# cortes-ciriano-lab/DeMethify

Measured on AMD Instinct MI355X. Metric: NMF update iters/sec (1e6 CpG x 256 samples x 16 types), higher is better.
Workload: dtype f64; 1 GPU; headline_1e6x256_12+4; N_cpg=1000000, S_samples=256, n_known=12, n_unknown=4, inner_iters=20, restarts=64, restart_seed=1 + k, restart_placement=k mod n_gpus, parallelism=restart-sharded x1

## Files before the change

### demethify_amd/csrc/dmf_api_solver.hip

```cpp
#include "dmf_api.h"

namespace dmf_api {

using dmf::kSplitInnerSteps;

static int ensure_split_scratch(dmf_solver* s, int n_iter2) {
    dmf_context* ctx = s->ctx;
    if (s->cm == nullptr) HIP_TRY(s->cm.alloc(ctx, (size_t)dmf::u_phase_split_cm_doubles(s->p->N, (int)s->n_u)));
    if (s->beta_cap < n_iter2 || s->beta_tab == nullptr) {
        s->beta_cap = n_iter2 > 0 ? n_iter2 : 1;
        HIP_TRY(s->beta_tab.alloc(ctx, (size_t)s->beta_cap));
    }
    return DMF_OK;
}

int enqueue_u_phase(dmf_solver* s, int n_iter2, dmf::RowKind row) {
    dmf_context* ctx = s->ctx;
    const dmf::ProblemView pv = s->p->view();
    FamilyScope scope(ctx, DMF_KERNEL_ROWPASS);
    switch (row) {
        case dmf::RowKind::CmI8InnerRows:
            DMF_TRY(ensure_split_scratch(s, n_iter2));
            HIP_TRY(dmf::launch_u_phase_split_i8(pv, s->iterate(), n_iter2, s->scratch(), ctx->stream));
            return DMF_OK;
// ... 171 lines not shown
    state->mom_i = 0;
    state->mom_n = n;
}

static double momentum_advance(double& a) {
#pragma clang fp contract(off)
    const double a0 = a;
    const double sq = 4.0 * a0 * a0;
    a = (1.0 + std::sqrt(1.0 + sq)) / 2.0;
    return (a0 - 1.0) / a;
}

static int upload_momentum_rows(dmf_solver* s, int rows, int n) {
    dmf_context* ctx = s->ctx;
    const int stride = 2 + 2 * n;
    if (s->mom_host == nullptr) {
        if (!ctx->pinned_moms.empty()) {
            s->mom_host = ctx->pinned_moms.back();
            ctx->pinned_moms.pop_back();
        } else {
            HIP_TRY(hipHostMalloc((void**)&s->mom_host, (size_t)kMomRows * (2 + 2 * kMomSteps) * sizeof(double)));
        }
        HIP_TRY(s->mom_dev.alloc(ctx, (size_t)kMomRows * (2 + 2 * kMomSteps)));
    }
    double a1 = s->h_state->a1, a2 = s->h_state->a2;
    for (int r = 0; r < rows; ++r) {
        double* row = s->mom_host + (size_t)r * stride;
        for (int t = 0; t < n; ++t) {
            row[2 + t] = momentum_advance(a1);
            row[2 + n + t] = momentum_advance(a2);
        }
        row[0] = a1;
        row[1] = a2;
    }
    HIP_TRY(hipMemcpyAsync(s->mom_dev, s->mom_host, (size_t)rows * stride * sizeof(double), hipMemcpyHostToDevice, ctx->stream));
    hipLaunchKernelGGL(k_set_momentum, dim3(1), dim3(1), 0, ctx->stream, s->state.get(), (const double*)s->mom_dev.get(), stride,
                       rows, n);
    HIP_TRY(hipGetLastError());
    return DMF_OK;
}

__global__ void k_set_tol(SolverState* state, double tol, double band) {
    state->tol = tol;
    state->band = band;
}

constexpr double kConfirmBand = 10.0;
constexpr double kGramCostRelErr = 1e-15;

static double* cost_slot(const dmf_solver* s) {
    return reinterpret_cast<double*>(reinterpret_cast<char*>(s->h_state) + kPinnedStateBytes - 16);
}

static int solver_setup(dmf_solver* s, const double* u0, const double* alpha0, int flags) {
    dmf_context* ctx = s->ctx;
    const dmf_problem* p = s->p;
    const int64_t N = p->N, S = p->S, n_c = p->n_c, n_u = s->n_u, K = n_c + n_u;
    dmf::ShapeKey& key = s->key;
    key.N = N;
    key.S = (int)S;
    key.n_c = (int)n_c;
    key.n_u = (int)n_u;
    key.nd = (p->ND > 0 && p->D16 != nullptr) ? p->ND : 0;
    key.SD = p->SD;
    key.x16 = key.nd > 0 && p->X16 != nullptr;
    key.rowpass_pair = ctx->rowpass_pair;
    key.level = ctx->generic_level;
    key.d_f32_exact = p->d_f32_exact;
    key.rtp_present = n_c == 0 || p->Rtp != nullptr;
    key.v_align = (unsigned)(reinterpret_cast<uintptr_t>(p->V.get()) & 15);
    key.rtp_align = (unsigned)(reinterpret_cast<uintptr_t>(p->Rtp.get()) & 15);
    key.alpha_unit = true;
    s->spec = dmf::select_path(key);
    if ((s->spec.use_v2 || s->spec.use_cm_i8) && !(flags & DMF_INIT_IN_UNIT_RANGE)) {
        bool in_unit = true;
        if (flags & DMF_PTR_DEVICE) {
            double outside = 0.0;
            HIP_TRY(dmf::launch_unit_range_check(alpha0, K * S, ctx->scratch, ctx->scratch + 2048, ctx->stream));
            HIP_TRY(hipMemcpyAsync(&outside, ctx->scratch + 2048, sizeof(double), hipMemcpyDeviceToHost, ctx->stream));
            HIP_TRY(hipStreamSynchronize(ctx->stream));
            in_unit = outside == 0.0;
        } else {
            for (int64_t i = 0; i < K * S; ++i)
                if (!(alpha0[i] >= 0.0 && alpha0[i] <= 1.0)) {
                    in_unit = false;
                    break;
                }
        }
        if (!in_unit) {
            key.alpha_unit = false;
            s->spec = dmf::select_path(key);
        }
    }
    if (!s->spec.supported) return DMF_ERR_UNSUPPORTED;
    s->in_flight = true;
    s->jobs.build((int)n_c, (int)K, [n_c, K](int k, int l) {
        if (l == (int)K && k < (int)n_c) return false;
        return !(l == (int)K && k == (int)K);
    });
    const int n_jobs = s->jobs.n;
    s->slab_doubles = dmf::gram_slab_doubles(N, (int)S, n_jobs);
    if (s->spec.use_gram_spec) {
        const int64_t spec = dmf::gram_u_slab_doubles(N, (int)S, (int)n_c, (int)n_u);
        if (spec > s->slab_doubles) s->slab_doubles = spec;
    }
    if (s->spec.use_gram_mfma) {
        const int64_t need = dmf::gram_mfma_slab_doubles(N, (int)S, n_jobs);
        if (need > s->slab_doubles) s->slab_doubles = need;
    }
    if (s->spec.use_fused) {
        const int64_t spec = dmf::rowpass_fused_slab_doubles(N - (N & 15), (int)S, (int)n_c, (int)n_u) +
                             dmf::gram_u_slab_doubles(16, (int)S, (int)n_c, (int)n_u);
        if (spec > s->slab_doubles) s->slab_doubles = spec;
    }
    if (s->spec.use_v2) {
        const int64_t bu = (int64_t)dmf::rowpass_v2_grid(N, (int)S) * n_u * S;
        if (bu > s->slab_doubles) s->slab_doubles = bu;
    }
    if (s->spec.use_gram_i8) {
        const int64_t bu = (int64_t)dmf::bu_cols_grid(N) * n_u * S;
        if (bu > s->slab_doubles) s->slab_doubles = bu;
        if (s->spec.use_cm_i8) {
            const int64_t bu2 = (int64_t)dmf::u_inner_bu_grid(N, (int)S) * n_u * S;
            if (bu2 > s->slab_doubles) s->slab_doubles = bu2;
        }
    }
    const size_t un = (size_t)N * n_u, an = (size_t)K * S;
    const size_t un_alloc = (un + 1) & ~(size_t)1;
    const size_t gbn = (size_t)(K + 1) * (K + 2) / 2 * S;
    const int nb_alpha = (int)((S + 63) / 64);
    HIP_TRY(s->u.alloc(ctx, un_alloc));
    HIP_TRY(s->u_prev.alloc(ctx, un_alloc));
    if (s->spec.u_path == 2) HIP_TRY(s->u_next.alloc(ctx, un_alloc));
    HIP_TRY(s->alpha.alloc(ctx, an));
    HIP_TRY(s->alpha_prev.alloc(ctx, an));
    HIP_TRY(s->gb.alloc(ctx, gbn));
    HIP_TRY(s->slab.alloc(ctx, (size_t)s->slab_doubles));
    HIP_TRY(s->partials.alloc(ctx, (size_t)2 * (nb_alpha + S)));
    HIP_TRY(s->u2_partials.alloc(ctx, 4096));
    if (s->spec.use_v2 || s->spec.use_gram_i8) {
        s->slab_i8_words = dmf::gram_i8_slab_words(N, p->SD, (int)n_c, (int)n_u);
        HIP_TRY(s->slab_i8.alloc(ctx, (size_t)s->slab_i8_words));
        const size_t acc_words = (size_t)dmf::gram_i8_acc_words((int)S, (int)n_c, (int)n_u);
        HIP_TRY(s->acc_i8.alloc(ctx, acc_words));
        HIP_TRY(hipMemsetAsync(s->acc_i8, 0, acc_words * sizeof(long long), ctx->stream));
    }
    HIP_TRY(s->state.alloc(ctx, 1));
    if (!ctx->pinned_states.empty()) {
        s->h_state = (SolverState*)ctx->pinned_states.back();
        ctx->pinned_states.pop_back();
    } else {
        HIP_TRY(hipHostMalloc((void**)&s->h_state, kPinnedStateBytes));
    }
    const hipMemcpyKind in_kind = (flags & DMF_PTR_DEVICE) ? hipMemcpyDeviceToDevice : hipMemcpyHostToDevice;
    HIP_TRY(hipMemsetAsync(s->state, 0, sizeof(SolverState), ctx->stream));
    HIP_TRY(hipMemsetAsync(s->gb, 0, gbn * sizeof(double), ctx->stream));
    HIP_TRY(hipMemcpyAsync(s->u, u0, un * sizeof(double), in_kind, ctx->stream));
    HIP_TRY(hipMemcpyAsync(s->u_prev, s->u, un * sizeof(double), hipMemcpyDeviceToDevice, ctx->stream));
    HIP_TRY(hipMemcpyAsync(s->alpha, alpha0, an * sizeof(double), in_kind, ctx->stream));
    HIP_TRY(hipMemcpyAsync(s->alpha_prev, s->alpha, an * sizeof(double), hipMemcpyDeviceToDevice, ctx->stream));
    DMF_TRY(s->jobs.upload(ctx));
    HIP_TRY(dmf::launch_scatter_known_block(p->gb_known, s->gb, (int)n_c, (int)K, (int)S, ctx->stream));
    HIP_TRY(dmf::launch_sumsq_f64(s->u, N * n_u, ctx->scratch, &s->state->u_norm2, nullptr, ctx->stream));
    HIP_TRY(dmf::launch_init_state(s->state, p->consts, s->alpha, (int)S, (int)n_c, (int)n_u, ctx->stream));
    if (!(flags & DMF_PTR_DEVICE)) HIP_TRY(hipStreamSynchronize(ctx->stream));
    return DMF_OK;
}

}

using namespace dmf_api;

extern "C" {

int dmf_solver_create(dmf_context* ctx, const dmf_problem* p, const double* u0, const double* alpha0,
                      int64_t n_u, int mode, int flags, dmf_solver** out) {
    DMF_TRY(check_ctx(ctx));
    if (out == nullptr) return DMF_ERR_BAD_ARG;
    *out = nullptr;
    if (p == nullptr || u0 == nullptr || alpha0 == nullptr || n_u < 1) return DMF_ERR_BAD_ARG;
    if (mode != DMF_MODE_PARTIAL && mode != DMF_MODE_UNSUPERVISED) return DMF_ERR_BAD_ARG;
    if (p->n_c + n_u > dmf::kMaxK) return DMF_ERR_UNSUPPORTED;
    SolverPtr s(new (std::nothrow) dmf_solver());
    if (s == nullptr) return DMF_ERR_BAD_ARG;
    s->ctx = ctx;
    s->p = p;
    s->n_u = n_u;
    s->mode = mode;
    DMF_TRY(solver_setup(s.get(), u0, alpha0, flags));
    *out = s.release();
    return DMF_OK;
}

int dmf_solver_step(dmf_solver* s, int64_t n_outer, int64_t n_iter2, double tol,
                    int64_t* iters_done_total, int* converged) {
    if (s == nullptr || n_outer < 0 || n_iter2 < 0 || n_iter2 > (1 << 20)) return DMF_ERR_BAD_ARG;
    dmf_context* ctx = s->ctx;
    DMF_TRY(check_ctx(ctx));
    const dmf_problem* p = s->p;
    const double gram_err = kGramCostRelErr * (double)p->N * (double)p->S * p->h_consts[kDmax] +
                            (s->key.x16 ? p->x16_dev * p->x16_sum : 0.0);
    s->confirm_stops = tol > 0.0 && ctx->stop_confirmation != 2 && (ctx->stop_confirmation == 1 || gram_err >= tol / 20.0);
    hipLaunchKernelGGL(k_set_tol, dim3(1), dim3(1), 0, ctx->stream, s->state.get(), tol, s->confirm_stops ? kConfirmBand : 1.0);
    HIP_TRY(hipGetLastError());
    if (s->cf_pending && tol > 0.0 && n_outer > 0) {
        FamilyScope scope(ctx, DMF_KERNEL_COST);
        HIP_TRY(enqueue_cost(ctx, p->view(), s->u, s->alpha, (int)s->n_u, ctx->scratch + 1024, &s->state->cf));
        s->cf_pending = false;
        s->cf_stream_iter = -2;
    }
    DMF_TRY(fetch_state(s));
    if (s->cf_stream_iter == -2) {
        s->cf_stream = s->h_state->cf;
        s->cf_stream_iter = s->h_state->iters;
    }
    int64_t check_every = s->spec.u_path != 2 ? 8 : 1;
    if (tol == 0.0 && s->spec.u_path != 2) check_every = kMomRows;
    const long long iters0 = s->h_state->iters;
    const dmf::IterationPlan plan = dmf::plan_iteration(s->key, s->spec, (int)n_iter2, s->purity != nullptr);
    const bool use_mom = n_iter2 >= 1 && n_iter2 <= kMomSteps && plan.row == dmf::RowKind::RowpassV2 &&
                         plan.alpha == dmf::AlphaKind::PhaseRow16;
    if (!use_mom && s->h_state->mom_n >= 0) {
        hipLaunchKernelGGL(k_set_momentum, dim3(1), dim3(1), 0, ctx->stream, s->state.get(), (const double*)nullptr, 0, 0, -1);
        HIP_TRY(hipGetLastError());
    }
    while (s->h_state->iters - iters0 < n_outer && s->h_state->done != 1) {
        const int64_t left = n_outer - (s->h_state->iters - iters0);
        const int64_t batch = left < check_every ? left : check_every;
        if (use_mom) DMF_TRY(upload_momentum_rows(s, (int)batch, (int)n_iter2));
        for (int64_t b = 0; b < batch; ++b) DMF_TRY(enqueue_outer_iteration(s, (int)n_iter2));
        DMF_TRY(fetch_state(s));
        if (s->h_state->iters > iters0) s->cf_pending = false;
        if (s->h_state->done == 2) {
            double cs = 0.0;
            DMF_TRY(cost_to_host(ctx, p->view(), s->u, s->alpha, (int)s->n_u, &cs, true));
            bool stop;
            if (s->cf_stream_iter == s->h_state->iters - 1) {
                stop = std::fabs(cs - s->cf_stream) < tol;
                s->n_confirmed += 1;
            } else {
                stop = std::fabs(s->h_state->cf - s->h_state->cf_prev) < tol;
                s->n_unconfirmed += 1;
            }
            s->cf_stream = cs;
            s->cf_stream_iter = s->h_state->iters;
            s->h_state->done = stop ? 1 : 0;
            DMF_TRY(push_state(s));
            check_every = 1;
        } else if (s->spec.u_path != 2 && check_every < 64 && check_every > 1) {
            check_every *= 2;
        }
    }
    if (iters_done_total) *iters_done_total = s->h_state->iters;
    if (converged) *converged = s->h_state->done == 1;
    return DMF_OK;
}

int dmf_solver_set_purity(dmf_solver* s, const double* purity, int flags) {
    if (s == nullptr || purity == nullptr) return DMF_ERR_BAD_ARG;
    dmf_context* ctx = s->ctx;
    DMF_TRY(check_ctx(ctx));
    if (s->mode != DMF_MODE_PARTIAL) return DMF_ERR_BAD_ARG;
    const size_t bytes = (size_t)s->p->S * sizeof(double);
    if (s->purity == nullptr) HIP_TRY(s->purity.alloc(ctx, (size_t)s->p->S));
    const hipMemcpyKind kind = (flags & DMF_PTR_DEVICE) ? hipMemcpyDeviceToDevice : hipMemcpyHostToDevice;
    HIP_TRY(hipMemcpyAsync(s->purity, purity, bytes, kind, ctx->stream));
    HIP_TRY(hipStreamSynchronize(ctx->stream));
    return DMF_OK;
}

int dmf_solver_get(dmf_solver* s, int flags, double* out_u, double* out_alpha, double* out_cost,
                   int64_t* out_iters) {
    if (s == nullptr) return DMF_ERR_BAD_ARG;
    dmf_context* ctx = s->ctx;
    DMF_TRY(check_ctx(ctx));
    const dmf_problem* p = s->p;
    DMF_TRY(export_array(ctx, s->u, (size_t)p->N * s->n_u * sizeof(double), flags, out_u));
    DMF_TRY(export_array(ctx, s->alpha, (size_t)(p->n_c + s->n_u) * p->S * sizeof(double), flags, out_alpha));
    if (s->cf_pending && out_cost != nullptr) {
        FamilyScope scope(ctx, DMF_KERNEL_COST);
        HIP_TRY(enqueue_cost(ctx, p->view(), s->u, s->alpha, (int)s->n_u, ctx->scratch + 1024, &s->state->cf));
        s->cf_pending = false;
    }
    DMF_TRY(fetch_state(s));
    if (out_cost) *out_cost = s->h_state->cf;
    if (out_iters) *out_iters = s->h_state->iters;
    return DMF_OK;
}

int dmf_solver_cost(dmf_solver* s, double* out_cost) {
    if (s == nullptr || out_cost == nullptr) return DMF_ERR_BAD_ARG;
    DMF_TRY(check_ctx(s->ctx));
    return cost_to_host(s->ctx, s->p->view(), s->u, s->alpha, (int)s->n_u, out_cost, true);
}

int dmf_solver_cost_begin(dmf_solver* s) {
    if (s == nullptr) return DMF_ERR_BAD_ARG;
    dmf_context* ctx = s->ctx;
    DMF_TRY(check_ctx(ctx));
    if (s->cost_event == nullptr) {
        if (!ctx->events.empty()) {
            s->cost_event = ctx->events.back();
            ctx->events.pop_back();
        } else {
            HIP_TRY(hipEventCreateWithFlags(&s->cost_event, hipEventDisableTiming));
        }
    }
    DMF_TRY(cost_to_host(ctx, s->p->view(), s->u, s->alpha, (int)s->n_u, cost_slot(s), false));
    HIP_TRY(hipEventRecord(s->cost_event, ctx->stream));
    s->cost_pending = true;
    return DMF_OK;
}

int dmf_solver_cost_end(dmf_solver* s, double* out_cost) {
    if (s == nullptr || out_cost == nullptr || !s->cost_pending) return DMF_ERR_BAD_ARG;
    DMF_TRY(check_ctx(s->ctx));
    HIP_TRY(hipEventSynchronize(s->cost_event));
// ... 77 lines not shown
```

### demethify_amd/csrc/dmf_internal.h

```cpp
#pragma once
#include <hip/hip_runtime.h>
#include <stdint.h>

#include "dmf_select.h"

namespace dmf {

struct SolverState {
    double a1;
    double a2;
    double l_w;
    double l_w_prev;
    double l_h;
    double l_h_prev;
    double dsq;
    double rt_norm2;
    double u_norm2;
    double cf;
    double cf_prev;
    double tol;
    long long iters;
    double band;
    int done;
    int arrive;
    const double* mom;
    int mom_stride, mom_rows, mom_i, mom_n;
};

__device__ __forceinline__ const double* momentum_row(const SolverState* __restrict__ state, int n_iter2) {
    return (state->mom != nullptr && state->mom_n == n_iter2 && state->mom_i < state->mom_rows)
               ? state->mom + (int64_t)state->mom_i * state->mom_stride
               : nullptr;
}

__host__ __device__ inline int tri(int k, int l) { return l * (l + 1) / 2 + k; }

constexpr int kMaxK = 64;
constexpr int kGramChunk = 16;
constexpr int kRowsPerBlockU = 64;

struct GramJobTable {
    const short* k_idx;
    const short* l_idx;
    const int* dst_row;
    int count;
};

struct PercentilePlan {
    long long k_prev, k_next;
    double gamma;
    int from_top;
    int pad;
};

struct ProblemView {
    const double* V = nullptr;
    const double* D = nullptr;
    const unsigned short* D16 = nullptr;
    const unsigned short* X16 = nullptr;
    const signed char* Dt8 = nullptr;
    int64_t plane_stride = 0;
    int SD = 0, ND = 0;
    const double* Rt = nullptr;
    const double* Rtp = nullptr;
    int64_t N = 0;
    int S = 0, n_c = 0;
    unsigned v_align() const { return (unsigned)(reinterpret_cast<uintptr_t>(V) & 15); }
    ProblemView rows(int64_t first, int64_t count) const {
        ProblemView r;
        r.V = V + first * S;
        r.D = D + first * S;
        r.Rt = Rt ? Rt + first * n_c : nullptr;
        r.Rtp = Rtp ? Rtp + first * ((n_c + 3) / 4 * 4) : nullptr;
        r.N = count;
        r.S = S;
        r.n_c = n_c;
        return r;
    }
};

struct IterateView {
    double* u = nullptr;
    double* u_prev = nullptr;
    const double* alpha = nullptr;
    SolverState* state = nullptr;
    int n_u = 0, mode = 0;
    IterateView rows(int64_t first) const {
        IterateView r = *this;
        r.u = u + first * n_u;
        r.u_prev = u_prev + first * n_u;
        return r;
    }
};

struct AlphaView {
    const double* gb = nullptr;
    double* alpha = nullptr;
    double* alpha_prev = nullptr;
    const double* purity = nullptr;
    SolverState* state = nullptr;
    double* partials = nullptr;
    int S = 0, n_c = 0, n_u = 0;
};

struct UScratch {
    double* cm = nullptr;
    double* beta = nullptr;
    double* slab = nullptr;
    double* u2_partials = nullptr;
};


hipError_t launch_convert_counts(const long long* src, double* dst, int64_t n, hipStream_t st);
hipError_t launch_max_f64(const double* x, int64_t n, double* scratch, double* out, hipStream_t st);
hipError_t launch_f32_residual_max(const double* x, int64_t n, double* scratch, double* out, hipStream_t st);
hipError_t launch_int_count_max(const double* x, int64_t n, double* scratch, double* out, hipStream_t st);
hipError_t launch_unit_range_check(const double* x, int64_t n, double* scratch, double* out, hipStream_t st);
hipError_t launch_sumsq_f64(const double* x, int64_t n, double* scratch, double* out,
                            const int* done_flag, hipStream_t st);
hipError_t launch_pad_rows(const double* src, double* dst, int64_t n_rows, int width_src, int width_dst,
                           hipStream_t st);
hipError_t launch_index_range_check(const long long* idx, int64_t n_idx, int64_t n_src, unsigned int* flag, hipStream_t st);
hipError_t launch_gather_rows(const double* src, double* dst, const long long* idx, int64_t n_idx,
                              int64_t width, hipStream_t st);

hipError_t launch_cost(const ProblemView& p, const double* u, const double* alpha, int n_u, double* scratch, double* out,
                       hipStream_t st);

bool cost_cols_supported(int S, int n_c, int n_u);
bool cost_cols2_wide_supported(const ProblemView& p, int n_u);
hipError_t launch_cost_cols2_wide(const ProblemView& p, const double* u, const double* alpha, int n_u, double* scratch,
                                  double* out, hipStream_t st);
int vdv_cols_grid(int64_t N);
hipError_t launch_vdv_cols(const ProblemView& p, double* slab, double* out, hipStream_t st);
hipError_t launch_cost_cols(const ProblemView& p, const double* u, const double* alpha, int n_u, double* scratch, double* out,
                            hipStream_t st);

hipError_t launch_gram(const ProblemView& p, const double* u, int n_u, GramJobTable jobs, double* slab, int64_t slab_doubles,
                       double* gb, const int* done_flag, hipStream_t st);
int64_t gram_slab_doubles(int64_t N, int S, int n_jobs);
hipError_t launch_gram_reduce(const double* slab, int ny, int n_jobs, int S, const int* dst_row,
                              double* gb, const int* done_flag, hipStream_t st);
bool gram_u_supported(int n_c, int n_u);
int64_t gram_u_slab_doubles(int64_t N, int S, int n_c, int n_u);
hipError_t launch_gram_u(const ProblemView& p, const double* u, int n_u, double* slab, const int* done_flag, int* ny_out,
                         hipStream_t st);

hipError_t launch_u_phase_gram(const ProblemView& p, const IterateView& it, int n_iter2, hipStream_t st);
bool u_phase_gram_supported(int S, int n_c, int n_u);
bool u_phase_mfma_supported(int S, int n_c, int n_u);
hipError_t launch_u_phase_mfma(const ProblemView& p, const IterateView& it, int n_iter2, hipStream_t st);
bool rowpass_fused_supported(int S, int n_c, int n_u);
int rowpass_fused_grid(int64_t N, int S);
int64_t rowpass_fused_slab_doubles(int64_t N, int S, int n_c, int n_u);
hipError_t launch_rowpass_fused(const ProblemView& p, const IterateView& it, int n_iter2, const UScratch& scratch,
                                int* grid_out, hipStream_t st);
hipError_t launch_finish_u_norm(const double* u2_partials, int n, SolverState* state, hipStream_t st);
hipError_t launch_u_step_direct(const ProblemView& p, const IterateView& it, double* u_next, int t, hipStream_t st);
bool u_step_direct_supported(int S, int n_c, int n_u);

hipError_t launch_alpha(AlphaKind kind, const AlphaView& a, int n_iter2, hipStream_t st);
hipError_t launch_set_lh(SolverState* state, hipStream_t st);
hipError_t launch_project_simplex(const double* X, double* out, int K, int S, double z,
                                  hipStream_t st);
hipError_t launch_scatter_known_block(const double* gb_known, double* gb, int n_c, int K, int S,
                                      hipStream_t st);
hipError_t launch_init_state(SolverState* state, const double* consts, const double* alpha,
                             int S, int n_c, int n_u, hipStream_t st);

int64_t u_phase_split_cm_doubles(int64_t N, int n_u);
hipError_t launch_u_phase_split(const ProblemView& p, const IterateView& it, int n_iter2, const UScratch& scratch,
                                hipStream_t st);

bool cm_i8_supported(unsigned v_align, int S, int n_c, int n_u, int ND, int SD);
hipError_t launch_cm_i8(const ProblemView& p, const IterateView& it, double* cm, hipStream_t st);
hipError_t launch_u_phase_split_i8(const ProblemView& p, const IterateView& it, int n_iter2, const UScratch& scratch,
                                   hipStream_t st);

bool u_inner_bu_supported(unsigned v_align, int S, int SD, int n_u, int n_iter2);
int u_inner_bu_grid(int64_t N, int S);
hipError_t launch_u_phase_split_i8_bu(const ProblemView& p, const IterateView& it, int n_iter2, const UScratch& scratch,
                                      int* grid_out, hipStream_t st);

bool u_phase_big_supported(int S, int n_c, int n_u, int n_iter2);
hipError_t launch_u_phase_big(const ProblemView& p, const IterateView& it, int n_iter2, hipStream_t st);

hipError_t launch_gram_mfma(const ProblemView& p, const double* u, int n_u, GramJobTable jobs, int n_dense, double* slab,
                            int64_t slab_doubles, const int* done_flag, int* ny_out, hipStream_t st);
int64_t gram_mfma_slab_doubles(int64_t N, int S, int n_jobs);

hipError_t launch_gather_counts_int(const unsigned short* src16, const unsigned short* src_x16, const long long* idx,
                                    int64_t n_idx, int SD, int ND, unsigned short* D16, unsigned short* X16, int64_t N16,
                                    signed char* Dt8, int64_t plane_stride, unsigned int* max_out,
                                    unsigned long long* xsum_out, hipStream_t st);
constexpr double kX16MaxDev = 8.0 * 0x1p-53;
hipError_t launch_build_counts_int(const double* D, const double* V, int64_t N, int S, int ND, unsigned short* D16,
                                   unsigned short* X16, int64_t N16, int SD, signed char* Dt8, int64_t plane_stride,
                                   unsigned long long* x_stats, hipStream_t st);
hipError_t launch_build_dt8(const unsigned short* D16, int64_t N, int SD, int ND, signed char* Dt8, int64_t plane_stride,
                            hipStream_t st);
hipError_t launch_mask_problem(const double* srcV, const double* srcD, const unsigned short* src16,
                               const unsigned short* srcX, const unsigned char* bits, double* dstV, double* dstD,
                               unsigned short* dst16, unsigned short* dstX, unsigned short* W16, int64_t N, int64_t N16, int S,
                               int SD, unsigned long long* stats, hipStream_t st);
hipError_t launch_holdout_weights_f64(const unsigned char* bits, double* W, int64_t N, int S, hipStream_t st);
bool rowpass_v2_supported(int S, int n_c, int n_u, int n_iter2);
int rowpass_v2_grid(int64_t N, int S);
hipError_t launch_rowpass_v2(const ProblemView& p, const IterateView& it, int n_iter2, const UScratch& scratch, int* grid_out,
                             bool pair, bool* paired_out, hipStream_t st);
bool rowpass_v2_pair_fits(int S, int n_u, int n_iter2);
bool gram_i8_supported(int n_c, int n_u, int ND, int64_t N, int SD);
int64_t gram_i8_slab_words(int64_t N, int SD, int n_c, int n_u);
int64_t gram_i8_acc_words(int S, int n_c, int n_u);
bool gram_i8_known_supported(int n_c, int ND, int64_t N, int SD);
int64_t gram_i8_slab_words_nf(int64_t N, int SD, int nf);
int64_t gram_i8_acc_words_nf(int S, int nf, int n_bu);
hipError_t launch_gram_i8(const ProblemView& p, const double* u, int n_u, const short* feat_a, const short* feat_b, int NF,
                          long long* slab, int64_t slab_words, const int* done_flag, int* ny_out, hipStream_t st);
int bu_cols_grid(int64_t N);
hipError_t launch_bu_cols(const ProblemView& p, const double* u, int n_u, double* slab, const int* done_flag,
                          int* n_slabs_out, hipStream_t st, bool* with_vdv = nullptr);
hipError_t launch_gram_v2_reduce(const long long* slab_i8, int ny, int NF, int SD, const double* slab_bu, int n_bu_slabs,
                                 int n_u, int S, long long* acc_words, const int* dst_row, double* gb, const int* done_flag,
                                 const double* u2_partials, int n_u2, SolverState* state, hipStream_t st);

hipError_t launch_percentile_pair(const double* x, int64_t n, int64_t m, PercentilePlan p0, PercentilePlan p1,
                                  double* out0, double* out1, hipStream_t st);
int64_t percentile_max_replicates();

int wls_moments_grid(int64_t N);
int64_t wls_slab_doubles(int64_t N, int S, int K);
hipError_t launch_wls_moments(const ProblemView& p, const double* u, int n_u, int target_dv, double* slab, double* mom,
                              hipStream_t st);
hipError_t launch_nnls_intercept(const double* gb, const double* mom, int K, int S, double* out, int* status, hipStream_t st);

constexpr int kSvdMaxS = 512, kSvdMaxNc = 64, kSvdMaxRank = 64;
constexpr size_t kSvdMaxLds = 160 * 1024;
size_t svd_project_lds_bytes(int S, int rank);
struct SvdColumns {
    double sign[kSvdMaxRank], scale[kSvdMaxRank];
};
bool svd_supported(int S, int n_c, int rank);
int svd_gram_grid(int64_t N, int S);
int64_t svd_gram_slab_doubles(int64_t N, int S);
hipError_t launch_svd_gram(const ProblemView& p, const double* H1, double* slab, int* flags, double* C, hipStream_t st);
int64_t svd_project_slab_doubles(int64_t N, int rank);
hipError_t launch_svd_project(const ProblemView& p, const double* H1, const double* Es, int rank, double* T, double* slab,
                              double* norms, hipStream_t st);
hipError_t launch_svd_finish(double* T, int64_t N, int rank, const SvdColumns& cols, hipStream_t st);

}
```

### demethify_amd/csrc/dmf_kernels_alpha.hip

```cpp
#include "dmf_device.h"
#include "dmf_dispatch.h"
#include "dmf_internal.h"

namespace dmf {

template <int KMAX>
__device__ __forceinline__ void sort_desc(double (&x)[KMAX]) {
#pragma unroll
    for (int k = 2; k <= KMAX; k <<= 1) {
#pragma unroll
        for (int j = k >> 1; j > 0; j >>= 1) {
#pragma unroll
            for (int i = 0; i < KMAX; ++i) {
                const int l = i ^ j;
                if (l > i) {
                    const double lo = fmin(x[i], x[l]), hi = fmax(x[i], x[l]);
                    if ((i & k) == 0) { x[i] = hi; x[l] = lo; }
                    else { x[i] = lo; x[l] = hi; }
                }
            }
        }
    }
}

// ... 573 lines not shown

template <int J>
__device__ __forceinline__ void argmin_step(double& v, int& idx, int k) {
    const double ov = row_xor<J>(v, k);
    const int oi = row_xor<J>(idx, k);
    const bool take = ov < v || (ov == v && oi < idx);
    v = take ? ov : v;
    idx = take ? oi : idx;
}

__global__ __launch_bounds__(64) void k_alpha_frank_wolfe_row16(const double* __restrict__ gb,
                                                                double* __restrict__ alpha,
                                                                const double* __restrict__ purity,
                                                                const SolverState* __restrict__ state, int S, int K,
                                                                int n_u, int max_iter, double* __restrict__ partials) {
    if (state->done) return;
    const int lane = threadIdx.x;
    const int k = lane & 15, grp = lane >> 4, base = grp * 16;
    const int s = blockIdx.x * 4 + grp;
    const bool col_ok = s < S;
    const int sc = col_ok ? s : S - 1;
    const bool row_ok = k < K;
    const int kc = row_ok ? k : K - 1;
    const int n_c = K - n_u;
    const bool known = k < n_c, unknown = row_ok && !known;

    double Grow[16];
#pragma unroll
    for (int l = 0; l < 16; ++l) {
        const int lc = l < K ? l : K - 1;
        const int lo = kc < lc ? kc : lc, hi = kc < lc ? lc : kc;
        const double v = gb[(int64_t)tri(lo, hi) * S + sc];
        Grow[l] = (row_ok && l < K) ? v : 0.0;
    }
    const double bk = row_ok ? gb[(int64_t)tri(kc, K) * S + sc] : 0.0;
    const double pur = purity[sc];
    const double mass = known ? pur : 1.0 - pur;
    double a = row_ok ? alpha[(int64_t)kc * S + sc] : 0.0;

    for (int it = 0; it < max_iter; ++it) {
        double g4[4] = {-bk, 0.0, 0.0, 0.0};
        fmac_rowbcast_seq<0, 16, true, true>(g4, a, Grow);
        const double grad = (g4[0] + g4[1]) + (g4[2] + g4[3]);
        double v1 = known ? grad : INFINITY, v2 = unknown ? grad : INFINITY;
        int i1 = k, i2 = k;
        argmin_step<1>(v1, i1, k); argmin_step<2>(v1, i1, k); argmin_step<4>(v1, i1, k); argmin_step<8>(v1, i1, k);
        argmin_step<1>(v2, i2, k); argmin_step<2>(v2, i2, k); argmin_step<4>(v2, i2, k); argmin_step<8>(v2, i2, k);
        const double gamma = 2.0 / (double)(it + 2);
        const bool at_vertex = (known && k == i1) || (unknown && k == i2);
        const double vertex = at_vertex ? mass : 0.0;
        a = (1.0 - gamma) * a + gamma * vertex;
    }
    if (col_ok && row_ok) alpha[(int64_t)k * S + s] = a;
    double ga = 0.0;
#pragma unroll
    for (int l = 0; l < 16; ++l) ga = fma(Grow[l], __shfl(a, base + l, 64), ga);
    double part = col_ok ? fma(a, ga, -2.0 * a * bk) : 0.0;
    if (col_ok && k == 0) part += gb[(int64_t)tri(K, K) * S + sc];
    const double n2 = (col_ok && unknown) ? a * a : 0.0;
    store_partials(partials, wave_sum(part), wave_sum(n2));
}

template <class F>
static hipError_t dispatch_kmax(int K, F&& f) {
    if (K > 16) return f(std::integral_constant<int, 0>{});
    if (K > 8) return f(std::integral_constant<int, 16>{});
    return K > 4 ? f(std::integral_constant<int, 8>{}) : f(std::integral_constant<int, 4>{});
}

template <int KMAX>
static hipError_t launch_alpha_thread(const AlphaView& a, int n_iter2, hipStream_t st) {
    const int K = a.n_c + a.n_u, nb = (a.S + 63) / 64;
    if constexpr (KMAX > 0) {
        const size_t lds = (size_t)(K + 1) * (K + 2) / 2 * 64 * sizeof(double);
        const int in_lds = lds <= 150 * 1024;
        if (in_lds && lds > 48 * 1024) {
            const hipError_t e = raise_dynamic_lds<k_alpha_phase<KMAX>>(lds);
            if (e != hipSuccess) return e;
        }
        hipLaunchKernelGGL(k_alpha_phase<KMAX>, dim3(nb), dim3(64), in_lds ? lds : 0, st, a.gb, a.alpha, a.alpha_prev, a.state,
                           a.S, K, a.n_u, n_iter2, in_lds, a.partials);
    } else {
        hipLaunchKernelGGL(k_alpha_phase_dyn, dim3(nb), dim3(64), 0, st, a.gb, a.alpha, a.alpha_prev, a.state, a.S, K, a.n_u,
                           n_iter2, a.partials);
    }
    return launch_finish_iteration(a.partials, nb, a.state, n_iter2, st);
}

template <int G>
static hipError_t launch_alpha_lanes(const AlphaView& a, int n_iter2, hipStream_t st) {
    const int nb = (a.S * G + 63) / 64;
    hipLaunchKernelGGL(k_alpha_phase_lanes<G>, dim3(nb), dim3(64), 0, st, a.gb, a.alpha, a.alpha_prev, a.state, a.S,
                       a.n_c + a.n_u, a.n_u, n_iter2, a.partials);
    return launch_finish_iteration(a.partials, nb, a.state, n_iter2, st);
}

hipError_t launch_alpha(AlphaKind kind, const AlphaView& a, int n_iter2, hipStream_t st) {
    const int S = a.S, K = a.n_c + a.n_u, nb4 = (S + 3) / 4, nb64 = (S + 63) / 64;
    if (K < 1 || K > kMaxK) return hipErrorInvalidValue;
    switch (kind) {
        case AlphaKind::PhaseRow16:
            if (K > 16) break;
            hipLaunchKernelGGL(k_alpha_phase_row16, dim3(nb4), dim3(64), 0, st, a.gb, a.alpha, a.alpha_prev, a.state, S, K, a.n_u,
                               n_iter2, a.partials);
            return hipGetLastError();
        case AlphaKind::PhaseLanes:
            if (K <= 16) break;
            return K <= 32 ? launch_alpha_lanes<32>(a, n_iter2, st) : launch_alpha_lanes<64>(a, n_iter2, st);
        case AlphaKind::Phase:
            if (K > 16) break;
            return dispatch_kmax(K, [&](auto kmax) { return launch_alpha_thread<kmax>(a, n_iter2, st); });
        case AlphaKind::PhaseDyn:
            if (K <= 16) break;
            return launch_alpha_thread<0>(a, n_iter2, st);
        case AlphaKind::FrankWolfeRow16:
            if (K > 16 || a.n_c < 1 || a.purity == nullptr) break;
            hipLaunchKernelGGL(k_alpha_frank_wolfe_row16, dim3(nb4), dim3(64), 0, st, a.gb, a.alpha, a.purity, a.state, S, K,
                               a.n_u, n_iter2, a.partials);
            return launch_finish_iteration(a.partials, nb4, a.state, n_iter2, st);
        case AlphaKind::FrankWolfe:
            if (a.purity == nullptr) break;
            hipLaunchKernelGGL(k_alpha_frank_wolfe, dim3(nb64), dim3(64), 0, st, a.gb, a.alpha, a.purity, a.state, S, K, a.n_u,
                               n_iter2, a.partials);
            return launch_finish_iteration(a.partials, nb64, a.state, n_iter2, st);
    }
    return hipErrorInvalidValue;
}

template <int KMAX>
__global__ __launch_bounds__(64) void k_project(const double* __restrict__ X, double* __restrict__ out,
                                                int K, int S, double z) {
    const int s = blockIdx.x * 64 + threadIdx.x;
    if (s >= S) return;
    double x[KMAX];
#pragma unroll
    for (int k = 0; k < KMAX; ++k) x[k] = k < K ? X[(int64_t)k * S + s] : 0.0;
    project_column<KMAX>(x, K, z);
#pragma unroll
    for (int k = 0; k < KMAX; ++k)
        if (k < K) out[(int64_t)k * S + s] = x[k];
}

hipError_t launch_project_simplex(const double* X, double* out, int K, int S, double z,
                                  hipStream_t st) {
    const dim3 grid((S + 63) / 64), block(64);
    if (K < 1 || K > kMaxK) return hipErrorInvalidValue;
    return dispatch_kmax(K, [&](auto kmax) {
        if constexpr (kmax > 0) hipLaunchKernelGGL(k_project<kmax>, grid, block, 0, st, X, out, K, S, z);
        else hipLaunchKernelGGL(k_project_dyn, grid, block, 0, st, X, out, K, S, z);
        return hipGetLastError();
    });
}

__global__ __launch_bounds__(256) void k_scatter_known(const double* __restrict__ gb_known,
                                                       double* __restrict__ gb, int n_c, int K, int S) {
    const int s = blockIdx.x * 256 + threadIdx.x;
    if (s >= S) return;
    for (int l = 0; l <= n_c; ++l) {
        const int ld = l == n_c ? K : l;
        for (int k = 0; k <= l; ++k) {
            const int kd = k == n_c ? K : k;
            gb[(int64_t)tri(kd, ld) * S + s] = gb_known[(int64_t)tri(k, l) * S + s];
        }
    }
}

hipError_t launch_scatter_known_block(const double* gb_known, double* gb, int n_c, int K, int S,
                                      hipStream_t st) {
    hipLaunchKernelGGL(k_scatter_known, dim3((S + 255) / 256), dim3(256), 0, st, gb_known, gb, n_c, K, S);
    return hipGetLastError();
}

__global__ __launch_bounds__(256) void k_init_state(SolverState* __restrict__ state,
                                                    const double* __restrict__ consts,
                                                    const double* __restrict__ alpha, int S, int n_c,
                                                    int n_u) {
    __shared__ double red[4];
    double acc = 0.0;
    const double* A2 = alpha + (int64_t)n_c * S;
    for (int i = threadIdx.x; i < n_u * S; i += 256) acc = fma(A2[i], A2[i], acc);
    const double n2 = block_sum<256>(acc, red);
    if (threadIdx.x == 0) {
        const double dsq = consts[0], rt2 = consts[1];
        state->a1 = 1.0;
        state->a2 = 1.0;
        state->dsq = dsq;
        state->rt_norm2 = rt2;
        state->l_w = n2 * dsq;
        state->l_w_prev = state->l_w;
        state->l_h = (rt2 + state->u_norm2) * dsq;
        state->l_h_prev = state->l_h;
        state->cf = __longlong_as_double(0x7FF8000000000000ll);
        state->cf_prev = state->cf;
        state->tol = 0.0;
        state->band = 1.0;
        state->mom = nullptr;
        state->mom_n = -1;
        state->iters = 0;
        state->done = 0;
        state->arrive = 0;
    }
}

hipError_t launch_init_state(SolverState* state, const double* consts, const double* alpha, int S,
                             int n_c, int n_u, hipStream_t st) {
    hipLaunchKernelGGL(k_init_state, dim3(1), dim3(256), 0, st, state, consts, alpha, S, n_c, n_u);
    return hipGetLastError();
}

}
```

### demethify_amd/csrc/dmf_kernels_stream.hip

```cpp
#include "dmf_device.h"
#include "dmf_dispatch.h"
#include "dmf_internal.h"

namespace dmf {

__global__ __launch_bounds__(256) void k_convert_counts(const long long* __restrict__ src,
                                                        double* __restrict__ dst, int64_t n) {
    int64_t i = (int64_t)blockIdx.x * 256 + threadIdx.x;
    const int64_t stride = (int64_t)gridDim.x * 256;
    for (; i < n; i += stride) dst[i] = (double)src[i];
}

hipError_t launch_convert_counts(const long long* src, double* dst, int64_t n, hipStream_t st) {
    if (n <= 0) return hipSuccess;
    int blocks = (int)((n + 255) / 256 < 8192 ? (n + 255) / 256 : 8192);
    hipLaunchKernelGGL(k_convert_counts, dim3(blocks), dim3(256), 0, st, src, dst, n);
    return hipGetLastError();
}

template <int MODE>
__global__ __launch_bounds__(256) void k_reduce_partial(const double* __restrict__ x, int64_t n,
                                                        double* __restrict__ partial,
                                                        const int* __restrict__ done_flag) {
    __shared__ double red[4];
    if (done_flag != nullptr && *done_flag) return;
    double acc = MODE == 1 ? 0.0 : -INFINITY;
    int64_t i = (int64_t)blockIdx.x * 256 + threadIdx.x;
    const int64_t stride = (int64_t)gridDim.x * 256;
    for (; i < n; i += stride) {
        const double v = x[i];
        if (MODE == 1) acc = fma(v, v, acc);
        else if (MODE == 0) acc = fmax(acc, v);
        else if (MODE == 2) acc = fmax(acc, fabs(v - (double)(float)v));
        else if (MODE == 3) acc = fmax(acc, (v >= 0.0 && v == rint(v)) ? v : INFINITY);
        else acc = fmax(acc, (v >= 0.0 && v <= 1.0) ? 0.0 : 1.0);
    }
    const double tot = MODE == 1 ? block_sum<256>(acc, red) : block_max<256>(acc, red);
    if (threadIdx.x == 0) partial[blockIdx.x] = tot;
}

template <int MODE>
__global__ __launch_bounds__(256) void k_reduce_final(const double* __restrict__ partial, int n,
                                                      double* __restrict__ out,
                                                      const int* __restrict__ done_flag) {
    __shared__ double red[4];
    if (done_flag != nullptr && *done_flag) return;
    double acc = MODE == 1 ? 0.0 : -INFINITY;
    for (int i = threadIdx.x; i < n; i += 256) {
        if (MODE == 1) acc += partial[i];
        else acc = fmax(acc, partial[i]);
    }
    const double tot = MODE == 1 ? block_sum<256>(acc, red) : block_max<256>(acc, red);
    if (threadIdx.x == 0) *out = tot;
}

static inline int reduce_blocks(int64_t n) {
    int64_t b = (n + 255) / 256;
    if (b > 1024) b = 1024;
    if (b < 1) b = 1;
    return (int)b;
}

hipError_t launch_max_f64(const double* x, int64_t n, double* scratch, double* out, hipStream_t st) {
    const int nb = reduce_blocks(n);
    hipLaunchKernelGGL(k_reduce_partial<0>, dim3(nb), dim3(256), 0, st, x, n, scratch, (const int*)nullptr);
    hipLaunchKernelGGL(k_reduce_final<0>, dim3(1), dim3(256), 0, st, scratch, nb, out, (const int*)nullptr);
    return hipGetLastError();
}

hipError_t launch_f32_residual_max(const double* x, int64_t n, double* scratch, double* out, hipStream_t st) {
    const int nb = reduce_blocks(n);
    hipLaunchKernelGGL(k_reduce_partial<2>, dim3(nb), dim3(256), 0, st, x, n, scratch, (const int*)nullptr);
    hipLaunchKernelGGL(k_reduce_final<0>, dim3(1), dim3(256), 0, st, scratch, nb, out, (const int*)nullptr);
    return hipGetLastError();
}

hipError_t launch_int_count_max(const double* x, int64_t n, double* scratch, double* out, hipStream_t st) {
    const int nb = reduce_blocks(n);
    hipLaunchKernelGGL(k_reduce_partial<3>, dim3(nb), dim3(256), 0, st, x, n, scratch, (const int*)nullptr);
    hipLaunchKernelGGL(k_reduce_final<0>, dim3(1), dim3(256), 0, st, scratch, nb, out, (const int*)nullptr);
    return hipGetLastError();
}

hipError_t launch_unit_range_check(const double* x, int64_t n, double* scratch, double* out, hipStream_t st) {
    const int nb = reduce_blocks(n);
    hipLaunchKernelGGL(k_reduce_partial<4>, dim3(nb), dim3(256), 0, st, x, n, scratch, (const int*)nullptr);
    hipLaunchKernelGGL(k_reduce_final<0>, dim3(1), dim3(256), 0, st, scratch, nb, out, (const int*)nullptr);
    return hipGetLastError();
}

hipError_t launch_sumsq_f64(const double* x, int64_t n, double* scratch, double* out,
                            const int* done_flag, hipStream_t st) {
    const int nb = reduce_blocks(n);
    hipLaunchKernelGGL(k_reduce_partial<1>, dim3(nb), dim3(256), 0, st, x, n, scratch, done_flag);
    hipLaunchKernelGGL(k_reduce_final<1>, dim3(1), dim3(256), 0, st, scratch, nb, out, done_flag);
    return hipGetLastError();
}

__global__ __launch_bounds__(256) void k_gather_rows(const double* __restrict__ src,
                                                     double* __restrict__ dst,
                                                     const long long* __restrict__ idx,
                                                     int64_t n_idx, int64_t width) {
    const int wave = threadIdx.x >> 6, lane = threadIdx.x & 63;
    int64_t r = (int64_t)blockIdx.x * 4 + wave;
    const int64_t stride = (int64_t)gridDim.x * 4;
    for (; r < n_idx; r += stride) {
        const double* s = src + idx[r] * width;
        double* d = dst + r * width;
        for (int64_t c = lane; c < width; c += 64) d[c] = s[c];
    }
}

hipError_t launch_gather_rows(const double* src, double* dst, const long long* idx, int64_t n_idx,
                              int64_t width, hipStream_t st) {
    if (n_idx <= 0 || width <= 0) return hipSuccess;
    int64_t b = (n_idx + 3) / 4;
    if (b > 65536) b = 65536;
    hipLaunchKernelGGL(k_gather_rows, dim3((unsigned)b), dim3(256), 0, st, src, dst, idx, n_idx, width);
    return hipGetLastError();
}

__global__ __launch_bounds__(256) void k_index_range_check(const long long* __restrict__ idx, int64_t n_idx, int64_t n_src,
                                                           unsigned int* __restrict__ flag) {
    bool bad = false;
    for (int64_t r = (int64_t)blockIdx.x * 256 + threadIdx.x; r < n_idx; r += (int64_t)gridDim.x * 256) {
        const long long v = idx[r];
        bad = bad || v < 0 || v >= n_src;
    }
    if (__ballot(bad) != 0ull && (threadIdx.x & 63) == 0) atomicOr(flag, 1u);
}

hipError_t launch_index_range_check(const long long* idx, int64_t n_idx, int64_t n_src, unsigned int* flag, hipStream_t st) {
    hipError_t e = hipMemsetAsync(flag, 0, sizeof(unsigned int), st);
    if (e != hipSuccess) return e;
    int64_t b = (n_idx + 255) / 256;
    if (b > 1024) b = 1024;
    hipLaunchKernelGGL(k_index_range_check, dim3((unsigned)(b < 1 ? 1 : b)), dim3(256), 0, st, idx, n_idx, n_src, flag);
    return hipGetLastError();
}

__global__ __launch_bounds__(256) void k_pad_rows(const double* __restrict__ src, double* __restrict__ dst,
                                                  int64_t n_rows, int width_src, int width_dst) {
    int64_t e = (int64_t)blockIdx.x * 256 + threadIdx.x;
    const int64_t total = n_rows * width_dst, stride = (int64_t)gridDim.x * 256;
    for (; e < total; e += stride) {
        const int64_t r = e / width_dst;
        const int c = (int)(e - r * width_dst);
        dst[e] = c < width_src ? src[r * width_src + c] : 0.0;
    }
}

hipError_t launch_pad_rows(const double* src, double* dst, int64_t n_rows, int width_src, int width_dst,
                           hipStream_t st) {
    if (n_rows <= 0 || width_dst <= 0) return hipSuccess;
    int64_t b = (n_rows * width_dst + 255) / 256;
    if (b > 8192) b = 8192;
    hipLaunchKernelGGL(k_pad_rows, dim3((unsigned)b), dim3(256), 0, st, src, dst, n_rows, width_src, width_dst);
    return hipGetLastError();
}

__global__ __launch_bounds__(256) void k_cost(const double* __restrict__ V, const double* __restrict__ D,
                                              const double* __restrict__ Rt, const double* __restrict__ u,
                                              const double* __restrict__ alpha, int64_t N, int S,
                                              int n_c, int n_u, int alpha_in_lds,
                                              double* __restrict__ partial) {
    extern __shared__ double lds_dyn[];
    __shared__ double red[4];
    const int K = n_c + n_u;
    const double* A = alpha;
    if (alpha_in_lds) {
        for (int i = threadIdx.x; i < K * S; i += 256) lds_dyn[i] = alpha[i];
        __syncthreads();
        A = lds_dyn;
    }
    const int tpr = S < 256 ? S : 256;
    const int rows_per_tile = 256 / tpr;
    const int r = threadIdx.x / tpr, c = threadIdx.x - r * tpr;
    double acc = 0.0;
    if (r < rows_per_tile) {
        const int64_t stride = (int64_t)gridDim.x * rows_per_tile;
        for (int64_t i0 = (int64_t)blockIdx.x * rows_per_tile + r; i0 < N; i0 += 4 * stride) {
            int64_t row[4];
            double w[4];
#pragma unroll
            for (int x = 0; x < 4; ++x) {
                const int64_t i = i0 + x * stride;
                w[x] = i < N ? 1.0 : 0.0;
                row[x] = i < N ? i : N - 1;
            }
            for (int s = c; s < S; s += tpr) {
                double v[4], d[4], pred[4];
#pragma unroll
                for (int x = 0; x < 4; ++x) {
                    v[x] = V[row[x] * S + s];
                    d[x] = D[row[x] * S + s];
                    pred[x] = 0.0;
                }
                for (int k = 0; k < n_c; ++k) {
                    const double ak = A[k * S + s];
#pragma unroll
                    for (int x = 0; x < 4; ++x) pred[x] = fma(Rt[row[x] * n_c + k], ak, pred[x]);
                }
                for (int j = 0; j < n_u; ++j) {
                    const double aj = A[(n_c + j) * S + s];
#pragma unroll
                    for (int x = 0; x < 4; ++x) pred[x] = fma(u[row[x] * n_u + j], aj, pred[x]);
                }
#pragma unroll
                for (int x = 0; x < 4; ++x) {
                    const double e = v[x] - pred[x];
                    acc = fma(w[x] * d[x] * e, e, acc);
                }
            }
        }
    }
    const double tot = block_sum<256>(acc, red);
    if (threadIdx.x == 0) partial[blockIdx.x] = tot;
}

template <int NKC, int NU, bool D16>
__global__ __launch_bounds__(256) void k_cost_cols(const double* __restrict__ V, const void* __restrict__ Dv, int SD,
                                                   const double* __restrict__ Rtp, const double* __restrict__ u,
                                                   const double* __restrict__ alpha, int64_t N, int S, int n_c,
                                                   double* __restrict__ partial) {
    constexpr int NCT = 4 * NKC;
    constexpr int kRows = 8;
    __shared__ double red[4];
    const int wave = __builtin_amdgcn_readfirstlane(threadIdx.x >> 6), lane = threadIdx.x & 63;
    const int s = blockIdx.y * 64 + lane;
    const bool active = s < S;
    const int sc = active ? s : S - 1;
    double ak[NCT > 0 ? NCT : 1], aj[NU > 0 ? NU : 1];
#pragma unroll
    for (int k = 0; k < NCT; ++k) ak[k] = k < n_c ? alpha[(int64_t)k * S + sc] : 0.0;
#pragma unroll
    for (int j = 0; j < NU; ++j) aj[j] = alpha[(int64_t)(n_c + j) * S + sc];
    const double* __restrict__ Df = reinterpret_cast<const double*>(Dv);
    const unsigned short* __restrict__ Dh = reinterpret_cast<const unsigned short*>(Dv);
    double acc = 0.0;
    const int64_t stride = (int64_t)gridDim.x * 4;
    for (int64_t i0 = (int64_t)blockIdx.x * 4 + wave; i0 < N; i0 += kRows * stride) {
        double v[kRows], d[kRows];
        int64_t row[kRows];
#pragma unroll
        for (int x = 0; x < kRows; ++x) {
            const int64_t i = i0 + x * stride;
            row[x] = i < N ? i : N - 1;
            v[x] = V[row[x] * S + sc];
// ... 366 lines not shown
```

Baseline: 1812 outer iters/s.

## Fuse solver-creation memsets, copies, norm reduction and state init into two kernels

Measured after the change: 1809 outer iters/s. Within noise of the previous version (-0.1%).

```diff
diff --git a/demethify_amd/csrc/dmf_api_solver.hip b/demethify_amd/csrc/dmf_api_solver.hip
--- a/demethify_amd/csrc/dmf_api_solver.hip
+++ b/demethify_amd/csrc/dmf_api_solver.hip
@@ -347,17 +347,17 @@
     } else {
         HIP_TRY(hipHostMalloc((void**)&s->h_state, kPinnedStateBytes));
     }
-    const hipMemcpyKind in_kind = (flags & DMF_PTR_DEVICE) ? hipMemcpyDeviceToDevice : hipMemcpyHostToDevice;
-    HIP_TRY(hipMemsetAsync(s->state, 0, sizeof(SolverState), ctx->stream));
-    HIP_TRY(hipMemsetAsync(s->gb, 0, gbn * sizeof(double), ctx->stream));
-    HIP_TRY(hipMemcpyAsync(s->u, u0, un * sizeof(double), in_kind, ctx->stream));
-    HIP_TRY(hipMemcpyAsync(s->u_prev, s->u, un * sizeof(double), hipMemcpyDeviceToDevice, ctx->stream));
-    HIP_TRY(hipMemcpyAsync(s->alpha, alpha0, an * sizeof(double), in_kind, ctx->stream));
-    HIP_TRY(hipMemcpyAsync(s->alpha_prev, s->alpha, an * sizeof(double), hipMemcpyDeviceToDevice, ctx->stream));
+    const double *u_src = u0, *alpha_src = alpha0;
+    if (!(flags & DMF_PTR_DEVICE)) {
+        HIP_TRY(hipMemcpyAsync(s->u, u0, un * sizeof(double), hipMemcpyHostToDevice, ctx->stream));
+        HIP_TRY(hipMemcpyAsync(s->alpha, alpha0, an * sizeof(double), hipMemcpyHostToDevice, ctx->stream));
+        u_src = s->u, alpha_src = s->alpha;
+    }
     DMF_TRY(s->jobs.upload(ctx));
-    HIP_TRY(dmf::launch_scatter_known_block(p->gb_known, s->gb, (int)n_c, (int)K, (int)S, ctx->stream));
-    HIP_TRY(dmf::launch_sumsq_f64(s->u, N * n_u, ctx->scratch, &s->state->u_norm2, nullptr, ctx->stream));
-    HIP_TRY(dmf::launch_init_state(s->state, p->consts, s->alpha, (int)S, (int)n_c, (int)n_u, ctx->stream));
+    int n_partial = 0;
+    HIP_TRY(dmf::launch_setup_u(u_src, s->u, s->u_prev, N * n_u, ctx->scratch, &n_partial, ctx->stream));
+    HIP_TRY(dmf::launch_solver_init(s->state, p->consts, ctx->scratch, n_partial, p->gb_known, s->gb, alpha_src, s->alpha,
+                                    s->alpha_prev, (int)S, (int)n_c, (int)n_u, ctx->stream));
     if (!(flags & DMF_PTR_DEVICE)) HIP_TRY(hipStreamSynchronize(ctx->stream));
     return DMF_OK;
 }
diff --git a/demethify_amd/csrc/dmf_internal.h b/demethify_amd/csrc/dmf_internal.h
--- a/demethify_amd/csrc/dmf_internal.h
+++ b/demethify_amd/csrc/dmf_internal.h
@@ -163,10 +163,11 @@
 hipError_t launch_set_lh(SolverState* state, hipStream_t st);
 hipError_t launch_project_simplex(const double* X, double* out, int K, int S, double z,
                                   hipStream_t st);
-hipError_t launch_scatter_known_block(const double* gb_known, double* gb, int n_c, int K, int S,
-                                      hipStream_t st);
-hipError_t launch_init_state(SolverState* state, const double* consts, const double* alpha,
-                             int S, int n_c, int n_u, hipStream_t st);
+hipError_t launch_setup_u(const double* src, double* u, double* u_prev, int64_t n, double* partial, int* n_partial_out,
+                          hipStream_t st);
+hipError_t launch_solver_init(SolverState* state, const double* consts, const double* u2_partial, int n_partial,
+                              const double* gb_known, double* gb, const double* alpha0, double* alpha, double* alpha_prev,
+                              int S, int n_c, int n_u, hipStream_t st);
 
 int64_t u_phase_split_cm_doubles(int64_t N, int n_u);
 hipError_t launch_u_phase_split(const ProblemView& p, const IterateView& it, int n_iter2, const UScratch& scratch,
diff --git a/demethify_amd/csrc/dmf_kernels_alpha.hip b/demethify_amd/csrc/dmf_kernels_alpha.hip
--- a/demethify_amd/csrc/dmf_kernels_alpha.hip
+++ b/demethify_amd/csrc/dmf_kernels_alpha.hip
@@ -749,59 +749,62 @@
     });
 }
 
-__global__ __launch_bounds__(256) void k_scatter_known(const double* __restrict__ gb_known,
-                                                       double* __restrict__ gb, int n_c, int K, int S) {
-    const int s = blockIdx.x * 256 + threadIdx.x;
-    if (s >= S) return;
-    for (int l = 0; l <= n_c; ++l) {
-        const int ld = l == n_c ? K : l;
-        for (int k = 0; k <= l; ++k) {
-            const int kd = k == n_c ? K : k;
-            gb[(int64_t)tri(kd, ld) * S + s] = gb_known[(int64_t)tri(k, l) * S + s];
-        }
-    }
-}
-
-hipError_t launch_scatter_known_block(const double* gb_known, double* gb, int n_c, int K, int S,
-                                      hipStream_t st) {
-    hipLaunchKernelGGL(k_scatter_known, dim3((S + 255) / 256), dim3(256), 0, st, gb_known, gb, n_c, K, S);
-    return hipGetLastError();
-}
-
-__global__ __launch_bounds__(256) void k_init_state(SolverState* __restrict__ state,
-                                                    const double* __restrict__ consts,
-                                                    const double* __restrict__ alpha, int S, int n_c,
-                                                    int n_u) {
+__global__ __launch_bounds__(256) void k_solver_init(SolverState* __restrict__ state, const double* __restrict__ consts,
+                                                     const double* __restrict__ u2_partial, int n_partial,
+                                                     const double* __restrict__ gb_known, double* __restrict__ gb,
+                                                     const double* __restrict__ alpha0, double* alpha,
+                                                     double* __restrict__ alpha_prev, int S, int n_c, int n_u) {
     __shared__ double red[4];
+    const int K = n_c + n_u, n_rows = (K + 1) * (K + 2) / 2;
+    for (int row = blockIdx.x; row < n_rows; row += gridDim.x) {
+        int l = 0;
+        while ((l + 1) * (l + 2) / 2 <= row) ++l;
+        const int k = row - l * (l + 1) / 2;
+        const bool known = (k < n_c || k == K) && (l < n_c || l == K);
+        const double* __restrict__ src = gb_known + (int64_t)tri(k == K ? n_c : k, l == K ? n_c : l) * S;
+        for (int s = threadIdx.x; s < S; s += 256) gb[(int64_t)row * S + s] = known ? src[s] : 0.0;
+    }
+    const bool copy_alpha = alpha != alpha0;
+    for (int i = blockIdx.x * 256 + threadIdx.x; i < K * S; i += gridDim.x * 256) {
+        const double a = alpha0[i];
+        if (copy_alpha) alpha[i] = a;
+        alpha_prev[i] = a;
+    }
+    if (blockIdx.x != 0) return;
     double acc = 0.0;
-    const double* A2 = alpha + (int64_t)n_c * S;
+    for (int i = threadIdx.x; i < n_partial; i += 256) acc += u2_partial[i];
+    const double u2 = block_sum<256>(acc, red);
+    acc = 0.0;
+    const double* A2 = alpha0 + (int64_t)n_c * S;
     for (int i = threadIdx.x; i < n_u * S; i += 256) acc = fma(A2[i], A2[i], acc);
     const double n2 = block_sum<256>(acc, red);
     if (threadIdx.x == 0) {
+        long long* words = reinterpret_cast<long long*>(state);
+        for (size_t w = 0; w < sizeof(SolverState) / sizeof(long long); ++w) words[w] = 0;
         const double dsq = consts[0], rt2 = consts[1];
         state->a1 = 1.0;
         state->a2 = 1.0;
         state->dsq = dsq;
         state->rt_norm2 = rt2;
+        state->u_norm2 = u2;
         state->l_w = n2 * dsq;
         state->l_w_prev = state->l_w;
-        state->l_h = (rt2 + state->u_norm2) * dsq;
+        state->l_h = (rt2 + u2) * dsq;
         state->l_h_prev = state->l_h;
         state->cf = __longlong_as_double(0x7FF8000000000000ll);
         state->cf_prev = state->cf;
-        state->tol = 0.0;
         state->band = 1.0;
-        state->mom = nullptr;
         state->mom_n = -1;
-        state->iters = 0;
-        state->done = 0;
-        state->arrive = 0;
-    }
-}
-
-hipError_t launch_init_state(SolverState* state, const double* consts, const double* alpha, int S,
-                             int n_c, int n_u, hipStream_t st) {
-    hipLaunchKernelGGL(k_init_state, dim3(1), dim3(256), 0, st, state, consts, alpha, S, n_c, n_u);
+    }
+}
+static_assert(sizeof(SolverState) % sizeof(long long) == 0, "k_solver_init zeroes the state in 8-byte words");
+
+hipError_t launch_solver_init(SolverState* state, const double* consts, const double* u2_partial, int n_partial,
+                              const double* gb_known, double* gb, const double* alpha0, double* alpha, double* alpha_prev,
+                              int S, int n_c, int n_u, hipStream_t st) {
+    const int K = n_c + n_u, n_rows = (K + 1) * (K + 2) / 2;
+    hipLaunchKernelGGL(k_solver_init, dim3(n_rows < 256 ? n_rows : 256), dim3(256), 0, st, state, consts, u2_partial, n_partial,
+                       gb_known, gb, alpha0, alpha, alpha_prev, S, n_c, n_u);
     return hipGetLastError();
 }
 
diff --git a/demethify_amd/csrc/dmf_kernels_stream.hip b/demethify_amd/csrc/dmf_kernels_stream.hip
--- a/demethify_amd/csrc/dmf_kernels_stream.hip
+++ b/demethify_amd/csrc/dmf_kernels_stream.hip
@@ -94,6 +94,31 @@
     const int nb = reduce_blocks(n);
     hipLaunchKernelGGL(k_reduce_partial<1>, dim3(nb), dim3(256), 0, st, x, n, scratch, done_flag);
     hipLaunchKernelGGL(k_reduce_final<1>, dim3(1), dim3(256), 0, st, scratch, nb, out, done_flag);
+    return hipGetLastError();
+}
+
+__global__ __launch_bounds__(256) void k_setup_u(const double* __restrict__ src, double* u, double* __restrict__ u_prev,
+                                                 int64_t n, double* __restrict__ partial) {
+    __shared__ double red[4];
+    const bool copy_u = u != src;
+    double acc = 0.0;
+    int64_t i = (int64_t)blockIdx.x * 256 + threadIdx.x;
+    const int64_t stride = (int64_t)gridDim.x * 256;
+    for (; i < n; i += stride) {
+        const double v = src[i];
+        if (copy_u) u[i] = v;
+        u_prev[i] = v;
+        acc = fma(v, v, acc);
+    }
+    const double tot = block_sum<256>(acc, red);
+    if (threadIdx.x == 0) partial[blockIdx.x] = tot;
+}
+
+hipError_t launch_setup_u(const double* src, double* u, double* u_prev, int64_t n, double* partial, int* n_partial_out,
+                          hipStream_t st) {
+    const int nb = reduce_blocks(n);
+    hipLaunchKernelGGL(k_setup_u, dim3(nb), dim3(256), 0, st, src, u, u_prev, n, partial);
+    *n_partial_out = nb;
     return hipGetLastError();
 }
 
```
